# ponimatkin/freepose

Measured on AMD Instinct MI355X. Metric: proposals/sec (ViT-L feat + top-k + 576-pose render-compare), higher is better.
Workload: dtype bf16

## Files before the change

freepose_amd/csrc/attention.hip:

```cpp
#include "internal.h"

#include <stdlib.h>

#include <type_traits>

namespace {

typedef __attribute__((ext_vector_type(2))) float f32x2_t;

constexpr int HD = 64;
constexpr int KVB = 64;
constexpr int QW = 32;
constexpr int NWAVE = 4;
constexpr int QB = QW * NWAVE;
constexpr int ROWB = 128;
constexpr int TILE = KVB * ROWB;
constexpr int STAGE = 2 * TILE;
constexpr float LAZY_THR = 40.0f;

struct AttnArgs {
    const bf16_t* QK; int ldqk;
    const bf16_t* Vt;
    bf16_t* O; int ldo;
    int B, H, n_tok, npad, D;
    float scale_log2e;
    int q_base;
};

__device__ __forceinline__ float vmax2(float a, float b) {
    float d;
    asm("v_max_f32 %0, %1, %2" : "=v"(d) : "v"(a), "v"(b));
    return d;
}
__device__ __forceinline__ float xlane_max16(float v) {
    const auto r = __builtin_amdgcn_permlane16_swap(__float_as_uint(v), __float_as_uint(v), false, false);
    return vmax2(__uint_as_float(r[0]), __uint_as_float(r[1]));
}
__device__ __forceinline__ float xlane_max32(float v) {
    const auto r = __builtin_amdgcn_permlane32_swap(__float_as_uint(v), __float_as_uint(v), false, false);
    return vmax2(__uint_as_float(r[0]), __uint_as_float(r[1]));
}
__device__ __forceinline__ int key_plain(int row) { return (row >> 1) & 7; }
__device__ __forceinline__ int key_krow(int row) { return ((((row >> 3) & 3) << 1) | ((row >> 1) & 1)) & 7; }
__device__ __forceinline__ int key_perm4(int row) {
    const int rl = row & 63;
    return (((rl >> 4) << 1) | ((rl & 3) >> 1)) & 7;
}

template <int NSLOT, int VAR = 0>
__global__ __launch_bounds__(NWAVE * 64, (VAR & 16) ? 4 : 3) void attn_fwd_kernel(AttnArgs p) {
    extern __shared__ __attribute__((aligned(1024))) char smem[];
    const int tid = threadIdx.x, lane = tid & 63;
    const int wave = __builtin_amdgcn_readfirstlane(tid >> 6);
    const int li = lane & 15, lg = lane >> 4;
    const int nqb = (p.npad - p.q_base + QB - 1) / QB;
    int bid = blockIdx.x;
    {
        const int nwg = gridDim.x;
        const int q = nwg >> 3, r = nwg & 7, xcd = bid & 7, pos = bid >> 3;
        bid = (xcd < r ? xcd * (q + 1) : r * (q + 1) + (xcd - r) * q) + pos;
    }
    const int qb = bid % nqb, bh = bid / nqb;
    const int h = bh % p.H, b = bh / p.H;
    const int q0 = p.q_base + qb * QB + wave * QW;
    const bool idle = q0 >= p.npad;

    const size_t rowbase = (size_t)b * p.npad;
    const char* gQK = (const char*)p.QK;
    const char* gVt = (const char*)(p.Vt + ((size_t)b * p.H + h) * HD * p.npad);

    bf16x8_t qf[2][2];
#pragma unroll
    for (int fq = 0; fq < 2; ++fq) {
        const int q = min(q0 + 16 * fq + li, p.npad - 1);
        const char* src = gQK + ((rowbase + q) * p.ldqk + h * HD) * 2;
#pragma unroll
        for (int kk = 0; kk < 2; ++kk) qf[fq][kk] = *(const bf16x8_t*)(src + (kk * 4 + lg) * 16);
    }

    uint32_t offK[2];
    int rowK[2];
    uint32_t offV[2];
    int slotV[2];
#pragma unroll
    for (int it = 0; it < 2; ++it) {
        const int row = (it * NWAVE + wave) * 8 + (lane >> 3);
        rowK[it] = row;
        offK[it] = (uint32_t)((p.D + h * HD) * 2 + (((lane & 7) ^ key_krow(row)) << 4));
        slotV[it] = (lane & 7) ^ key_perm4(row);
        offV[it] = (uint32_t)row * (uint32_t)p.npad * 2u;
    }
    const char* gKb = gQK + rowbase * (size_t)p.ldqk * 2;
    uint32_t lofK[2], lofV[2];
#pragma unroll
    for (int it = 0; it < 2; ++it) {
        lofK[it] = (uint32_t)rowK[it] * (uint32_t)p.ldqk * 2u + offK[it];
        lofV[it] = offV[it] + (uint32_t)(slotV[it] * 16);
    }
    const uint32_t kstep = (uint32_t)p.ldqk * 2u;
    auto stage = [&](int buf, int kv0) {
        char* sb = smem + buf * STAGE;
        if (kv0 + KVB <= p.npad) {
#pragma unroll
            for (int it = 0; it < 2; ++it) glds16_buf(gKb, lofK[it], (uint32_t)kv0 * kstep, sb + (it * NWAVE + wave) * 1024);
#pragma unroll
            for (int it = 0; it < 2; ++it) glds16_buf(gVt, lofV[it], (uint32_t)kv0 * 2u, sb + TILE + (it * NWAVE + wave) * 1024);
        } else {
#pragma unroll
            for (int it = 0; it < 2; ++it) {
                const int key = min(kv0 + rowK[it], p.npad - 1);
                glds16(gQK + (rowbase + key) * (size_t)p.ldqk * 2 + offK[it], sb + (it * NWAVE + wave) * 1024);
            }
#pragma unroll
            for (int it = 0; it < 2; ++it) {
                const int k8 = min(kv0 + slotV[it] * 8, p.npad - 8);
                glds16(gVt + offV[it] + (size_t)k8 * 2, sb + TILE + (it * NWAVE + wave) * 1024);
            }
        }
    };

    const int keyK = (((li >> 2) << 1) | ((li & 3) >> 1)) & 7;
    const int baseK = ((li >> 2) * 8 + (li & 3)) * ROWB;
    const int keyV = (((li >> 2) << 1) | ((li & 3) >> 1)) & 7;
    const int baseV = TILE + ((li >> 2) * 16 + (li & 3)) * ROWB;

    f32x4_t o[4][2];
#pragma unroll
    for (int i = 0; i < 4; ++i)
#pragma unroll
        for (int j = 0; j < 2; ++j) o[i][j] = f32x4_t{0.f, 0.f, 0.f, 0.f};
    float mrow[2] = {-1e30f, -1e30f};
    float mthr[2] = {-1e30f, -1e30f};
    float nmb[2] = {0.f, 0.f};
    constexpr bool PRE = (VAR & 64) != 0;
    constexpr bool VSUM = (VAR & 256) != 0;
    float vsum[2] = {0.f, 0.f};
    f32x4_t nref[2] = {f32x4_t{0.f, 0.f, 0.f, 0.f}, f32x4_t{0.f, 0.f, 0.f, 0.f}};
    f32x4_t lacc[2] = {f32x4_t{0.f, 0.f, 0.f, 0.f}, f32x4_t{0.f, 0.f, 0.f, 0.f}};
    bf16x8_t ones;
#pragma unroll
    for (int e = 0; e < 8; ++e) ones[e] = (__bf16)1.0f;

    const int ntile = (p.n_tok + KVB - 1) / KVB;
    constexpr bool SHORT = (VAR & 4) != 0;
    auto tile_of = [&](int sq) { return SHORT ? (sq == 0 ? ntile - 1 : sq - 1) : sq; };
    constexpr int PF = NSLOT - 1;
    stage(0, tile_of(0) * KVB);
#pragma unroll
    for (int i = 1; i < PF; ++i)
        if (ntile > i) stage(i, tile_of(i) * KVB);
    asm volatile("s_waitcnt vmcnt(0)" ::: "memory");
#pragma unroll
    for (int fq = 0; fq < 2; ++fq)
#pragma unroll
        for (int kk = 0; kk < 2; ++kk) asm volatile("" : "+v"(qf[fq][kk]));
    if constexpr (VAR & 2) {
        const int d = (blockIdx.x * 5) % 12;
        for (int i = 0; i < d; ++i) __builtin_amdgcn_s_sleep(2);
    }
    auto tile_body = [&](int t, auto slot_c, auto nks_c, auto first_c) {
        const int slot = slot_c;
        constexpr int NKS = decltype(nks_c)::value;
        constexpr bool FIRST = decltype(first_c)::value;
        const int ahead = min(PF - 1, ntile - 1 - t);
        if (ahead >= 2) asm volatile("s_waitcnt vmcnt(8)" ::: "memory");
        else if (ahead == 1) asm volatile("s_waitcnt vmcnt(4)" ::: "memory");
        else asm volatile("s_waitcnt vmcnt(0)" ::: "memory");
        __builtin_amdgcn_s_barrier();
        asm volatile("" ::: "memory");
        if (t + PF < ntile) stage(slot >= 1 ? slot - 1 : NSLOT - 1, tile_of(t + PF) * KVB);
        if (idle) return;
        const char* sb = smem + slot * STAGE;
        const int kv0 = tile_of(t) * KVB;

        f32x4_t s[4][2];
        if constexpr (VAR & 1) __builtin_amdgcn_s_setprio(1);
#pragma unroll
        for (int kk = 0; kk < 2; ++kk) {
            const int slot = (((kk << 2) | lg) ^ keyK) << 4;
#pragma unroll
            for (int fk = 0; fk < 2 * NKS; ++fk) {
                const bf16x8_t kf = *(const bf16x8_t*)(sb + baseK + (32 * (fk >> 1) + 4 * (fk & 1)) * ROWB + slot);
#pragma unroll
                for (int fq = 0; fq < 2; ++fq)
                    s[fk][fq] = __builtin_amdgcn_mfma_f32_16x16x32_bf16(kf, qf[fq][kk], kk == 0 ? (PRE ? nref[fq] : f32x4_t{0.f, 0.f, 0.f, 0.f}) : s[fk][fq], 0, 0, 0);
            }
        }
        if constexpr (VAR & 1) __builtin_amdgcn_s_setprio(0);
        if (kv0 + KVB > p.n_tok) {
#pragma unroll
            for (int fk = 0; fk < 2 * NKS; ++fk)
#pragma unroll
                for (int r = 0; r < 4; ++r)
                    if (kv0 + 32 * (fk >> 1) + 8 * lg + 4 * (fk & 1) + r >= p.n_tok) {
                        s[fk][0][r] = -1e30f;
                        s[fk][1][r] = -1e30f;
                    }
        }

        constexpr bool JITV = (VAR & 16) != 0;
        bf16x8_t vf[JITV ? 1 : 2][4];
        if constexpr (!JITV) {
#pragma unroll
        for (int ks = 0; ks < NKS; ++ks) {
            const int sv = (((ks << 2) | lg) ^ keyV) << 4;
#pragma unroll
            for (int fd = 0; fd < 4; ++fd) vf[ks][fd] = *(const bf16x8_t*)(sb + baseV + fd * 4 * ROWB + sv);
        }
        }

        bf16x8_t pf[2][2];
        auto softmax_max = [&](int fq) {
            float mx;
            if constexpr (NKS == 1)
                asm("v_max3_f32 %0, %1, %2, %3\n\tv_max3_f32 %0, %0, %4, %5\n\tv_max3_f32 %0, %0, %6, %7\n\tv_max_f32 %0, %0, %8"
                    : "=&v"(mx)
                    : "v"(s[0][fq][0]), "v"(s[0][fq][1]), "v"(s[0][fq][2]), "v"(s[0][fq][3]), "v"(s[1][fq][0]), "v"(s[1][fq][1]),
                      "v"(s[1][fq][2]), "v"(s[1][fq][3]));
            else
            asm("v_max3_f32 %0, %1, %2, %3\n\tv_max3_f32 %0, %0, %4, %5\n\tv_max3_f32 %0, %0, %6, %7\n\tv_max3_f32 %0, %0, %8, %9\n\t"
                "v_max3_f32 %0, %0, %10, %11\n\tv_max3_f32 %0, %0, %12, %13\n\tv_max3_f32 %0, %0, %14, %15\n\tv_max_f32 %0, %0, %16"
                : "=&v"(mx)
                : "v"(s[0][fq][0]), "v"(s[0][fq][1]), "v"(s[0][fq][2]), "v"(s[0][fq][3]), "v"(s[1][fq][0]), "v"(s[1][fq][1]),
                  "v"(s[1][fq][2]), "v"(s[1][fq][3]), "v"(s[2][fq][0]), "v"(s[2][fq][1]), "v"(s[2][fq][2]), "v"(s[2][fq][3]),
                  "v"(s[3][fq][0]), "v"(s[3][fq][1]), "v"(s[3][fq][2]), "v"(s[3][fq][3]));
            if constexpr (PRE) {
                constexpr float THR2 = LAZY_THR * 1.4426950408889634f / 8.0f;
                if (FIRST || __builtin_amdgcn_ballot_w64(mx > THR2) != 0) {
                    mx = xlane_max16(mx);
                    mx = xlane_max32(mx);
                    const float delta = FIRST ? mx : vmax2(mx, 0.f);
#pragma unroll
                    for (int r = 0; r < 4; ++r) nref[fq][r] -= delta;
#pragma unroll
                    for (int fk = 0; fk < 2 * NKS; ++fk)
#pragma unroll
                        for (int r = 0; r < 4; ++r) s[fk][fq][r] -= delta;
                    if constexpr (!FIRST) {
                        const float alpha = __builtin_amdgcn_exp2f(-delta);
                        lacc[fq][0] *= alpha;
                        if constexpr (VSUM) vsum[fq] *= alpha;
#pragma unroll
                        for (int fd = 0; fd < 4; ++fd)
#pragma unroll
                            for (int r = 0; r < 4; ++r) o[fd][fq][r] *= alpha;
                    }
                }
            } else
            if (__builtin_amdgcn_ballot_w64(mx > mthr[fq]) != 0) {
                mx = xlane_max16(mx);
                mx = xlane_max32(mx);
                const float mnew = vmax2(mrow[fq], mx);
                const float alpha = __builtin_amdgcn_exp2f((mrow[fq] - mnew) * p.scale_log2e);
                mrow[fq] = mnew;
                mthr[fq] = mnew + LAZY_THR;
                nmb[fq] = -(mnew * p.scale_log2e);
                lacc[fq][0] *= alpha;
#pragma unroll
                for (int fd = 0; fd < 4; ++fd)
#pragma unroll
                    for (int r = 0; r < 4; ++r) o[fd][fq][r] *= alpha;
            }
        };
        auto softmax_exp = [&](int fq) {
            float pv[4][4];
            if constexpr (PRE) {
#pragma unroll
                for (int fk = 0; fk < 2 * NKS; ++fk)
#pragma unroll
                    for (int r = 0; r < 4; ++r) pv[fk][r] = __builtin_amdgcn_exp2f(s[fk][fq][r]);
            } else if constexpr (VAR & 128) {
                const f32x2_t sc2 = {p.scale_log2e, p.scale_log2e};
                const f32x2_t mb2 = {nmb[fq], nmb[fq]};
#pragma unroll
                for (int fk = 0; fk < 2 * NKS; ++fk)
#pragma unroll
                    for (int r = 0; r < 4; r += 2) {
                        const f32x2_t a = {s[fk][fq][r], s[fk][fq][r + 1]};
                        const f32x2_t e = __builtin_elementwise_fma(a, sc2, mb2);
                        pv[fk][r] = __builtin_amdgcn_exp2f(e[0]);
                        pv[fk][r + 1] = __builtin_amdgcn_exp2f(e[1]);
                    }
            } else {
#pragma unroll
                for (int fk = 0; fk < 2 * NKS; ++fk)
#pragma unroll
                    for (int r = 0; r < 4; ++r) {
                        float e;
                        asm("v_fma_f32 %0, %1, %2, %3" : "=v"(e) : "v"(s[fk][fq][r]), "v"(p.scale_log2e), "v"(nmb[fq]));
                        pv[fk][r] = __builtin_amdgcn_exp2f(e);
                    }
            }
#pragma unroll
            for (int ks = 0; ks < NKS; ++ks) {
                uint4 w;
                w.x = pack_bf2(pv[2 * ks][0], pv[2 * ks][1]);
                w.y = pack_bf2(pv[2 * ks][2], pv[2 * ks][3]);
                w.z = pack_bf2(pv[2 * ks + 1][0], pv[2 * ks + 1][1]);
                w.w = pack_bf2(pv[2 * ks + 1][2], pv[2 * ks + 1][3]);
                pf[fq][ks] = __builtin_bit_cast(bf16x8_t, w);
            }
        };
        auto pv_half = [&](int fq) {
#pragma unroll
            for (int ks = 0; ks < NKS; ++ks) {
#pragma unroll
                for (int fd = 0; fd < 4; ++fd)
                    o[fd][fq] = __builtin_amdgcn_mfma_f32_16x16x32_bf16(vf[JITV ? 0 : ks][fd], pf[fq][ks], o[fd][fq], 0, 0, 0);
                lacc[fq] = __builtin_amdgcn_mfma_f32_16x16x32_bf16(ones, pf[fq][ks], lacc[fq], 0, 0, 0);
            }
        };

        if constexpr (JITV) {
            softmax_max(0);
            softmax_exp(0);
            softmax_max(1);
            softmax_exp(1);
#pragma unroll
            for (int ks = 0; ks < NKS; ++ks) {
                const int sv = (((ks << 2) | lg) ^ keyV) << 4;
#pragma unroll
                for (int fd = 0; fd < 4; ++fd) vf[0][fd] = *(const bf16x8_t*)(sb + baseV + fd * 4 * ROWB + sv);
#pragma unroll
                for (int fq = 0; fq < 2; ++fq) {
#pragma unroll
                    for (int fd = 0; fd < 4; ++fd)
                        o[fd][fq] = __builtin_amdgcn_mfma_f32_16x16x32_bf16(vf[0][fd], pf[fq][ks], o[fd][fq], 0, 0, 0);
                    if constexpr (VSUM) {
                        typedef __bf16 bf16x2_hw __attribute__((ext_vector_type(2)));
                        const uint4 pw = __builtin_bit_cast(uint4, pf[fq][ks]);
                        const bf16x2_hw one2 = __builtin_bit_cast(bf16x2_hw, 0x3f803f80u);
                        vsum[fq] = __builtin_amdgcn_fdot2_f32_bf16(__builtin_bit_cast(bf16x2_hw, pw.x), one2, vsum[fq], false);
                        vsum[fq] = __builtin_amdgcn_fdot2_f32_bf16(__builtin_bit_cast(bf16x2_hw, pw.y), one2, vsum[fq], false);
                        vsum[fq] = __builtin_amdgcn_fdot2_f32_bf16(__builtin_bit_cast(bf16x2_hw, pw.z), one2, vsum[fq], false);
                        vsum[fq] = __builtin_amdgcn_fdot2_f32_bf16(__builtin_bit_cast(bf16x2_hw, pw.w), one2, vsum[fq], false);
                    } else {
                        lacc[fq] = __builtin_amdgcn_mfma_f32_16x16x32_bf16(ones, pf[fq][ks], lacc[fq], 0, 0, 0);
                    }
                }
            }
            return;
        }
        softmax_max(0);
        softmax_exp(0);
        softmax_max(1);
        __builtin_amdgcn_sched_barrier(0);
        softmax_exp(1);
        pv_half(0);
#pragma unroll
        for (int g = 0; g < 5 * NKS; ++g) {
            __builtin_amdgcn_sched_group_barrier(0x008, 1, 0);
            __builtin_amdgcn_sched_group_barrier(0x002, 4, 0);
        }
        __builtin_amdgcn_sched_barrier(0);
        if constexpr (VAR & 1) __builtin_amdgcn_s_setprio(1);
        pv_half(1);
        if constexpr (VAR & 1) __builtin_amdgcn_s_setprio(0);
    };
    using full_c = std::integral_constant<int, 2>;
    using half_c = std::integral_constant<int, 1>;
    using yes_c = std::true_type;
    using no_c = std::false_type;
    if constexpr (SHORT) {
        static_assert(NSLOT == 2, "the short-tail prologue is written for the 2-slot ring");
        tile_body(0, std::integral_constant<int, 0>{}, half_c{}, yes_c{});
        for (int t = 1; t < ntile; t += 2) {
            tile_body(t, std::integral_constant<int, 1>{}, full_c{}, no_c{});
            if (t + 1 < ntile) tile_body(t + 1, std::integral_constant<int, 0>{}, full_c{}, no_c{});
        }
    } else if constexpr (NSLOT == 2 && PRE) {
        tile_body(0, std::integral_constant<int, 0>{}, full_c{}, yes_c{});
        for (int t = 1; t < ntile; t += 2) {
            tile_body(t, std::integral_constant<int, 1>{}, full_c{}, no_c{});
            if (t + 1 < ntile) tile_body(t + 1, std::integral_constant<int, 0>{}, full_c{}, no_c{});
        }
    } else if constexpr (NSLOT == 2) {
        for (int t = 0; t < ntile; t += 2) {
            tile_body(t, std::integral_constant<int, 0>{}, full_c{}, no_c{});
            if (t + 1 < ntile) tile_body(t + 1, std::integral_constant<int, 1>{}, full_c{}, no_c{});
        }
    } else {
        tile_body(0, 0, full_c{}, yes_c{});
        int slot = NSLOT > 1 ? 1 : 0;
        for (int t = 1; t < ntile; ++t) {
            tile_body(t, slot, full_c{}, no_c{});
            slot = slot + 1 == NSLOT ? 0 : slot + 1;
        }
    }

#pragma unroll
    for (int fq = 0; fq < 2; ++fq) {
        float rowsum = lacc[fq][0];
        if constexpr (VSUM) {
            rowsum = vsum[fq];
            rowsum += lane_xor<16>(rowsum);
            rowsum += lane_xor<32>(rowsum);
        }
        const float inv = 1.0f / rowsum;
        const int q = q0 + 16 * fq + li;
        if (q < p.npad) {
            uint4 w0, w1;
            w0.x = pack_bf2(o[0][fq][0] * inv, o[0][fq][1] * inv);
            w0.y = pack_bf2(o[0][fq][2] * inv, o[0][fq][3] * inv);
            w0.z = pack_bf2(o[1][fq][0] * inv, o[1][fq][1] * inv);
            w0.w = pack_bf2(o[1][fq][2] * inv, o[1][fq][3] * inv);
            w1.x = pack_bf2(o[2][fq][0] * inv, o[2][fq][1] * inv);
            w1.y = pack_bf2(o[2][fq][2] * inv, o[2][fq][3] * inv);
            w1.z = pack_bf2(o[3][fq][0] * inv, o[3][fq][1] * inv);
            w1.w = pack_bf2(o[3][fq][2] * inv, o[3][fq][3] * inv);
            uint4* dst = (uint4*)(p.O + (rowbase + q) * p.ldo + h * HD + lg * 16);
            dst[0] = w0;
            dst[1] = w1;
        }
    }
}

}

int fp_attention_fwd(const bf16_t* QK, int ldqk, const bf16_t* Vt, bf16_t* O, int ldo, int B, int H,
                     int n_tok, int npad, bool q_prescaled, hipStream_t stream) {
    FP_REQUIRE(B > 0 && H > 0 && n_tok > 0 && npad >= n_tok && npad % 16 == 0,
               "attention: bad shape B=%d H=%d n_tok=%d npad=%d", B, H, n_tok, npad);
    FP_REQUIRE(npad >= 8, "attention: npad too small");
    AttnArgs a;
    a.QK = QK; a.ldqk = ldqk; a.Vt = Vt; a.O = O; a.ldo = ldo;
    a.B = B; a.H = H; a.n_tok = n_tok; a.npad = npad; a.D = H * HD;
    a.scale_log2e = FP_ATTN_QSCALE;
    a.q_base = 0;
    dim3 grid(cdiv(npad - a.q_base, QB) * H * B);
    const bool short_tail = n_tok > KVB && n_tok - (cdiv(n_tok, KVB) - 1) * KVB <= KVB / 2;
#ifdef FP_LAB
    const int nslot = fp_opt_get(FP_OPT_ATTN_SLOTS, 2);
    static int env_var = [] { const char* e = getenv("FP_ATTN_VARIANT"); return e ? atoi(e) : 0; }();
    const int avar = fp_opt_get(FP_OPT_ATTN_VARIANT, env_var);
    if (!q_prescaled) {
    if (nslot == 2 && (avar & 2)) { hipLaunchKernelGGL((attn_fwd_kernel<2, 2>), grid, dim3(NWAVE * 64), 2 * STAGE, stream, a); FP_LAUNCH_CHECK(); return FP_OK; }
    if (nslot == 2 && (avar & 1)) { hipLaunchKernelGGL((attn_fwd_kernel<2, 1>), grid, dim3(NWAVE * 64), 2 * STAGE, stream, a); FP_LAUNCH_CHECK(); return FP_OK; }
    if (nslot == 4) { hipLaunchKernelGGL(attn_fwd_kernel<4>, grid, dim3(NWAVE * 64), 4 * STAGE, stream, a); FP_LAUNCH_CHECK(); return FP_OK; }
    if (nslot == 3) { hipLaunchKernelGGL(attn_fwd_kernel<3>, grid, dim3(NWAVE * 64), 3 * STAGE, stream, a); FP_LAUNCH_CHECK(); return FP_OK; }
    if (avar & 8) { hipLaunchKernelGGL(attn_fwd_kernel<2>, grid, dim3(NWAVE * 64), 2 * STAGE, stream, a); FP_LAUNCH_CHECK(); return FP_OK; }
    if ((avar & 128) && !q_prescaled) {
        if (short_tail) hipLaunchKernelGGL((attn_fwd_kernel<2, 4 | 16 | 128>), grid, dim3(NWAVE * 64), 2 * STAGE, stream, a);
        else hipLaunchKernelGGL((attn_fwd_kernel<2, 16 | 128>), grid, dim3(NWAVE * 64), 2 * STAGE, stream, a);
        FP_LAUNCH_CHECK();
        return FP_OK;
    }
    if (avar & 32) {
        if (short_tail) hipLaunchKernelGGL((attn_fwd_kernel<2, 4>), grid, dim3(NWAVE * 64), 2 * STAGE, stream, a);
        else hipLaunchKernelGGL(attn_fwd_kernel<2>, grid, dim3(NWAVE * 64), 2 * STAGE, stream, a);
        FP_LAUNCH_CHECK();
        return FP_OK;
    }
    }
#endif
#ifdef FP_LAB
    if (q_prescaled && (fp_opt_get(FP_OPT_ATTN_VARIANT, 0) & 256)) {
        if (short_tail) hipLaunchKernelGGL((attn_fwd_kernel<2, 4 | 16 | 64 | 256>), grid, dim3(NWAVE * 64), 2 * STAGE, stream, a);
        else hipLaunchKernelGGL((attn_fwd_kernel<2, 16 | 64 | 256>), grid, dim3(NWAVE * 64), 2 * STAGE, stream, a);
        FP_LAUNCH_CHECK();
        return FP_OK;
    }
#endif
    if (q_prescaled) {
        if (short_tail) hipLaunchKernelGGL((attn_fwd_kernel<2, 4 | 16 | 64>), grid, dim3(NWAVE * 64), 2 * STAGE, stream, a);
        else hipLaunchKernelGGL((attn_fwd_kernel<2, 16 | 64>), grid, dim3(NWAVE * 64), 2 * STAGE, stream, a);
    } else {
        if (short_tail) hipLaunchKernelGGL((attn_fwd_kernel<2, 4 | 16>), grid, dim3(NWAVE * 64), 2 * STAGE, stream, a);
        else hipLaunchKernelGGL((attn_fwd_kernel<2, 16>), grid, dim3(NWAVE * 64), 2 * STAGE, stream, a);
    }
    FP_LAUNCH_CHECK();
    return FP_OK;
}
```

Before: 1.983.

## Add row-sum overflow guard to lazy-rescale attention, recompute tile on overflow

Adds a GUARD variant (VAR bit 512) and makes it the default for the pre-scaled path. For non-first tiles it skips the per-tile max/ballot rescale check: it exponentiates, accumulates row sums, and only if a sum overflows (not below 2^64) restores the old sum and recomputes QK with a forced max rescale. The K staging also reuses one offset register with a shifted base, and the tail path recomputes addresses to save registers. The gamble is that overflow is rare, so the common path is cheaper, while an overflowing tile pays for a second QK pass.

```diff
diff --git a/freepose_amd/csrc/attention.hip b/freepose_amd/csrc/attention.hip
--- a/freepose_amd/csrc/attention.hip
+++ b/freepose_amd/csrc/attention.hip
@@ -102,9 +102,28 @@
         char* sb = smem + buf * STAGE;
         if (kv0 + KVB <= p.npad) {
 #pragma unroll
-            for (int it = 0; it < 2; ++it) glds16_buf(gKb, lofK[it], (uint32_t)kv0 * kstep, sb + (it * NWAVE + wave) * 1024);
+            for (int it = 0; it < 2; ++it) {
+                if constexpr ((VAR & 512) != 0) glds16_buf(gKb, lofK[0], (uint32_t)(kv0 + 32 * it) * kstep, sb + (it * NWAVE + wave) * 1024);
+                else glds16_buf(gKb, lofK[it], (uint32_t)kv0 * kstep, sb + (it * NWAVE + wave) * 1024);
+            }
 #pragma unroll
             for (int it = 0; it < 2; ++it) glds16_buf(gVt, lofV[it], (uint32_t)kv0 * 2u, sb + TILE + (it * NWAVE + wave) * 1024);
+        } else if constexpr ((VAR & 512) != 0) {
+            int ln = lane;
+            asm volatile("" : "+v"(ln));
+#pragma unroll
+            for (int it = 0; it < 2; ++it) {
+                const int row = (it * NWAVE + wave) * 8 + (ln >> 3);
+                const int key = min(kv0 + row, p.npad - 1);
+                const uint32_t ok = (uint32_t)((p.D + h * HD) * 2 + (((ln & 7) ^ key_krow(row)) << 4));
+                glds16(gQK + (rowbase + key) * (size_t)p.ldqk * 2 + ok, sb + (it * NWAVE + wave) * 1024);
+            }
+#pragma unroll
+            for (int it = 0; it < 2; ++it) {
+                const int row = (it * NWAVE + wave) * 8 + (ln >> 3);
+                const int k8 = min(kv0 + ((ln & 7) ^ key_perm4(row)) * 8, p.npad - 8);
+                glds16(gVt + (size_t)row * p.npad * 2 + (size_t)k8 * 2, sb + TILE + (it * NWAVE + wave) * 1024);
+            }
         } else {
 #pragma unroll
             for (int it = 0; it < 2; ++it) {
@@ -134,6 +153,8 @@
     float nmb[2] = {0.f, 0.f};
     constexpr bool PRE = (VAR & 64) != 0;
     constexpr bool VSUM = (VAR & 256) != 0;
+    constexpr bool GUARD = (VAR & 512) != 0;
+    static_assert(!GUARD || ((VAR & (16 | 64)) == (16 | 64) && !VSUM), "the row-sum guard is written for the pre-scaled four-wave flavour");
     float vsum[2] = {0.f, 0.f};
     f32x4_t nref[2] = {f32x4_t{0.f, 0.f, 0.f, 0.f}, f32x4_t{0.f, 0.f, 0.f, 0.f}};
     f32x4_t lacc[2] = {f32x4_t{0.f, 0.f, 0.f, 0.f}, f32x4_t{0.f, 0.f, 0.f, 0.f}};
@@ -174,6 +195,7 @@
         const int kv0 = tile_of(t) * KVB;
 
         f32x4_t s[4][2];
+        auto qk_products = [&]() {
         if constexpr (VAR & 1) __builtin_amdgcn_s_setprio(1);
 #pragma unroll
         for (int kk = 0; kk < 2; ++kk) {
@@ -197,6 +219,8 @@
                         s[fk][1][r] = -1e30f;
                     }
         }
+        };
+        qk_products();
 
         constexpr bool JITV = (VAR & 16) != 0;
         bf16x8_t vf[JITV ? 1 : 2][4];
@@ -210,7 +234,8 @@
         }
 
         bf16x8_t pf[2][2];
-        auto softmax_max = [&](int fq) {
+        auto softmax_max = [&](int fq, auto force_c) {
+            constexpr bool FORCE = decltype(force_c)::value;
             float mx;
             if constexpr (NKS == 1)
                 asm("v_max3_f32 %0, %1, %2, %3\n\tv_max3_f32 %0, %0, %4, %5\n\tv_max3_f32 %0, %0, %6, %7\n\tv_max_f32 %0, %0, %8"
@@ -226,7 +251,7 @@
                   "v"(s[3][fq][0]), "v"(s[3][fq][1]), "v"(s[3][fq][2]), "v"(s[3][fq][3]));
             if constexpr (PRE) {
                 constexpr float THR2 = LAZY_THR * 1.4426950408889634f / 8.0f;
-                if (FIRST || __builtin_amdgcn_ballot_w64(mx > THR2) != 0) {
+                if (FIRST || FORCE || __builtin_amdgcn_ballot_w64(mx > THR2) != 0) {
                     mx = xlane_max16(mx);
                     mx = xlane_max32(mx);
                     const float delta = FIRST ? mx : vmax2(mx, 0.f);
@@ -311,10 +336,58 @@
             }
         };
 
+        if constexpr (GUARD && !FIRST) {
+            softmax_exp(0);
+            softmax_exp(1);
+            float lold[2];
+#pragma unroll
+            for (int fq = 0; fq < 2; ++fq) asm("v_mov_b32 %0, %1" : "=v"(lold[fq]) : "v"(lacc[fq][0]));
+            auto row_sums = [&]() {
+#pragma unroll
+                for (int ks = 0; ks < NKS; ++ks)
+#pragma unroll
+                    for (int fq = 0; fq < 2; ++fq) lacc[fq] = __builtin_amdgcn_mfma_f32_16x16x32_bf16(ones, pf[fq][ks], lacc[fq], 0, 0, 0);
+            };
+            auto read_vt = [&](int ks) {
+                const int sv = (((ks << 2) | lg) ^ keyV) << 4;
+#pragma unroll
+                for (int fd = 0; fd < 4; ++fd) vf[0][fd] = *(const bf16x8_t*)(sb + baseV + fd * 4 * ROWB + sv);
+            };
+            row_sums();
+            read_vt(0);
+            constexpr float LMAX = 18446744073709551616.0f;
+            const bool fired = __builtin_amdgcn_ballot_w64(!(lacc[0][0] < LMAX) || !(lacc[1][0] < LMAX)) != 0;
+#pragma unroll
+            for (int fd = 0; fd < 4; ++fd) asm volatile("" : "+v"(vf[0][fd]));
+            if (fired) {
+                asm volatile("" ::: "memory");
+#pragma unroll
+                for (int fq = 0; fq < 2; ++fq)
+#pragma unroll
+                    for (int r = 0; r < 4; ++r) lacc[fq][r] = lold[fq];
+                qk_products();
+                softmax_max(0, std::true_type{});
+                softmax_exp(0);
+                softmax_max(1, std::true_type{});
+                softmax_exp(1);
+                row_sums();
+                read_vt(0);
+            }
+#pragma unroll
+            for (int ks = 0; ks < NKS; ++ks) {
+                if (ks) read_vt(ks);
+#pragma unroll
+                for (int fq = 0; fq < 2; ++fq)
+#pragma unroll
+                    for (int fd = 0; fd < 4; ++fd)
+                        o[fd][fq] = __builtin_amdgcn_mfma_f32_16x16x32_bf16(vf[0][fd], pf[fq][ks], o[fd][fq], 0, 0, 0);
+            }
+            return;
+        }
         if constexpr (JITV) {
-            softmax_max(0);
+            softmax_max(0, std::false_type{});
             softmax_exp(0);
-            softmax_max(1);
+            softmax_max(1, std::false_type{});
             softmax_exp(1);
 #pragma unroll
             for (int ks = 0; ks < NKS; ++ks) {
@@ -341,9 +414,9 @@
             }
             return;
         }
-        softmax_max(0);
+        softmax_max(0, std::false_type{});
         softmax_exp(0);
-        softmax_max(1);
+        softmax_max(1, std::false_type{});
         __builtin_amdgcn_sched_barrier(0);
         softmax_exp(1);
         pv_half(0);
@@ -388,6 +461,9 @@
         }
     }
 
+    int ln = lane;
+    if constexpr (GUARD) asm volatile("" : "+v"(ln));
+    const int li_s = ln & 15, lg_s = ln >> 4;
 #pragma unroll
     for (int fq = 0; fq < 2; ++fq) {
         float rowsum = lacc[fq][0];
@@ -397,7 +473,7 @@
             rowsum += lane_xor<32>(rowsum);
         }
         const float inv = 1.0f / rowsum;
-        const int q = q0 + 16 * fq + li;
+        const int q = q0 + 16 * fq + li_s;
         if (q < p.npad) {
             uint4 w0, w1;
             w0.x = pack_bf2(o[0][fq][0] * inv, o[0][fq][1] * inv);
@@ -408,7 +484,7 @@
             w1.y = pack_bf2(o[2][fq][2] * inv, o[2][fq][3] * inv);
             w1.z = pack_bf2(o[3][fq][0] * inv, o[3][fq][1] * inv);
             w1.w = pack_bf2(o[3][fq][2] * inv, o[3][fq][3] * inv);
-            uint4* dst = (uint4*)(p.O + (rowbase + q) * p.ldo + h * HD + lg * 16);
+            uint4* dst = (uint4*)(p.O + (rowbase + q) * p.ldo + h * HD + lg_s * 16);
             dst[0] = w0;
             dst[1] = w1;
         }
@@ -454,6 +530,12 @@
     }
 #endif
 #ifdef FP_LAB
+    if (q_prescaled && (fp_opt_get(FP_OPT_ATTN_VARIANT, 0) & 512)) {
+        if (short_tail) hipLaunchKernelGGL((attn_fwd_kernel<2, 4 | 16 | 64>), grid, dim3(NWAVE * 64), 2 * STAGE, stream, a);
+        else hipLaunchKernelGGL((attn_fwd_kernel<2, 16 | 64>), grid, dim3(NWAVE * 64), 2 * STAGE, stream, a);
+        FP_LAUNCH_CHECK();
+        return FP_OK;
+    }
     if (q_prescaled && (fp_opt_get(FP_OPT_ATTN_VARIANT, 0) & 256)) {
         if (short_tail) hipLaunchKernelGGL((attn_fwd_kernel<2, 4 | 16 | 64 | 256>), grid, dim3(NWAVE * 64), 2 * STAGE, stream, a);
         else hipLaunchKernelGGL((attn_fwd_kernel<2, 16 | 64 | 256>), grid, dim3(NWAVE * 64), 2 * STAGE, stream, a);
@@ -462,8 +544,8 @@
     }
 #endif
     if (q_prescaled) {
-        if (short_tail) hipLaunchKernelGGL((attn_fwd_kernel<2, 4 | 16 | 64>), grid, dim3(NWAVE * 64), 2 * STAGE, stream, a);
-        else hipLaunchKernelGGL((attn_fwd_kernel<2, 16 | 64>), grid, dim3(NWAVE * 64), 2 * STAGE, stream, a);
+        if (short_tail) hipLaunchKernelGGL((attn_fwd_kernel<2, 4 | 16 | 64 | 512>), grid, dim3(NWAVE * 64), 2 * STAGE, stream, a);
+        else hipLaunchKernelGGL((attn_fwd_kernel<2, 16 | 64 | 512>), grid, dim3(NWAVE * 64), 2 * STAGE, stream, a);
     } else {
         if (short_tail) hipLaunchKernelGGL((attn_fwd_kernel<2, 4 | 16>), grid, dim3(NWAVE * 64), 2 * STAGE, stream, a);
         else hipLaunchKernelGGL((attn_fwd_kernel<2, 16>), grid, dim3(NWAVE * 64), 2 * STAGE, stream, a);
```

New measurement: 1.998, median of 6. Within noise of the previous version (+0.7%).
